# hpcaitech/Open-Sora

Hardware: NVIDIA H100
Metric: denoise-steps/sec STDiT3-XL/2 64x32x32 bf16 (higher is better)
Workload: dtype bf16

## Files before the change

### open-sora_b200/csrc/gemm_sm90.cu

```cuda
#include <stdlib.h>

#include <type_traits>

#include "common.cuh"
#include "tiles.cuh"
#include "wgmma.cuh"

namespace osb {

constexpr int kBlockM = 128;
constexpr int kBlockK = 64;
constexpr int kNumThreads = 384;
constexpr int kStageBudget = 200 * 1024;
constexpr int kSmemLimit = 227 * 1024;

enum { kPlain = 0, kConv = 1, kHeadTiles = 2, kLora = 3, kText = 4, kFp8 = 5, kFp8Blk = 6 };

struct Fp8BlockParams {
  int64_t a_ld, a_kstride;
  uint8_t* d8;
  float* d_scale;
  int64_t ldd8, ld_dscale;
};

// ... 13 lines not shown
struct HeadTileParams {
  uint8_t* base;
  int64_t kind_stride, head_stride;
  TileMap map;
  int32_t tile_bytes;
  int32_t heads, nkinds;
  uint32_t norm_mask, rope_mask;
  const __nv_bfloat16* norm_w[4];
  float eps;
  const float* cos;
  const float* sin;
};

struct ConvGeom {
  int32_t wt_log2, ht_log2;
  int32_t tiles_w, tiles_h, tiles_t, nb;
  int32_t w_out, h_out, t_out;
  int32_t sw, sh, st;
  int32_t kw_n, kh_n;
  int32_t cin_chunks;
};

__host__ __device__ constexpr bool staged_epilogue(int mode) { return mode == kPlain || mode == kConv || mode == kLora || mode == kFp8 || mode == kFp8Blk; }

template <int BLOCK_N, bool kStaged = false>
struct GemmCfg {
  static constexpr int A_BYTES = kBlockM * kBlockK * 2;
  static constexpr int B_BYTES = BLOCK_N * kBlockK * 2;
  static constexpr int STAGE_BYTES = A_BYTES + B_BYTES;
  static constexpr int EPI_BYTES = kStaged ? kBlockM * BLOCK_N * 2 : 0;
  static constexpr int RING_BUDGET = kStaged ? kSmemLimit - 1024 - 256 - EPI_BYTES : kStageBudget;
  static constexpr int STAGES_RAW = RING_BUDGET / STAGE_BYTES;
  static constexpr int STAGES = STAGES_RAW > 6 ? 6 : STAGES_RAW;
  static constexpr int NUM_BARS = 2 * STAGES + (kStaged ? 1 : 0);
  static constexpr int SMEM_BYTES = STAGES * STAGE_BYTES + EPI_BYTES + 1024 + 8 * NUM_BARS;
  static_assert(STAGES >= 2, "pipeline needs at least two stages");
  static_assert(SMEM_BYTES <= kSmemLimit, "shared memory");
  static_assert(B_BYTES % 1024 == 0, "W tile must keep 1024-byte swizzle-atom alignment");
  static_assert(BLOCK_N % 16 == 0 && BLOCK_N <= 256, "wgmma N");
  static_assert(!kStaged || BLOCK_N % 64 == 0, "the staged epilogue moves 64-column boxes");
};

template <int BLOCK_N, int kMode>
__global__ void __launch_bounds__(kNumThreads, 1)
gemm_bf16_kernel(const __grid_constant__ CUtensorMap tmap_a, const __grid_constant__ CUtensorMap tmap_w,
                 const GemmEpilogueParams p, const ConvGeom cg, const HeadTileParams ht,
                 const __grid_constant__ CUtensorMap tmap_u, const __grid_constant__ CUtensorMap tmap_lb,
                 const int32_t lora_k_blocks,
                 const float* a_scale, const float* w_scale,
                 const Fp8BlockParams fb,
                 const __grid_constant__ CUtensorMap tmap_r,
                 const __grid_constant__ CUtensorMap tmap_d) {
  constexpr bool kStaged = staged_epilogue(kMode);
  using Cfg = GemmCfg<BLOCK_N, kStaged>;
  constexpr int kStages = Cfg::STAGES;
  constexpr int kBK = (kMode == kFp8 || kMode == kFp8Blk) ? 2 * kBlockK : kBlockK;
  constexpr uint32_t kEpiBoxBytes = kBlockM * 128;

  extern __shared__ uint8_t smem_raw[];
  const uint32_t smem_base = (smem_u32(smem_raw) + 1023u) & ~1023u;
  const uint32_t epi_base = smem_base + kStages * Cfg::STAGE_BYTES;
  const uint32_t bar_base = epi_base + Cfg::EPI_BYTES;
  auto full_bar = [&](int s) { return bar_base + 8u * s; };
  auto empty_bar = [&](int s) { return bar_base + 8u * (kStages + s); };
  const uint32_t res_bar = bar_base + 8u * (2 * kStages);
  auto smem_a = [&](int s) { return smem_base + s * Cfg::STAGE_BYTES; };
  auto smem_b = [&](int s) { return smem_base + s * Cfg::STAGE_BYTES + Cfg::A_BYTES; };

  const int wg = threadIdx.x >> 7;
  const int tid_wg = threadIdx.x & 127;
  const int64_t num_n_blocks = (p.N + BLOCK_N - 1) / BLOCK_N;
  const int64_t m_blk = blockIdx.x / num_n_blocks, n_blk = blockIdx.x % num_n_blocks;
  const int64_t num_k_blocks = (p.K + kBK - 1) / kBK;
  const int64_t total_k_blocks = kMode == kLora ? num_k_blocks + lora_k_blocks : num_k_blocks;
  int n_i = 0, t0 = 0, h0 = 0, w0 = 0;
  if constexpr (kMode == kConv) {
    const int tw = (int)(m_blk % cg.tiles_w);
    const int th = (int)((m_blk / cg.tiles_w) % cg.tiles_h);
    const int tt = (int)((m_blk / ((int64_t)cg.tiles_w * cg.tiles_h)) % cg.tiles_t);
    n_i = (int)(m_blk / ((int64_t)cg.tiles_w * cg.tiles_h * cg.tiles_t));
    w0 = tw << cg.wt_log2;
    h0 = th << cg.ht_log2;
    t0 = tt * (128 >> (cg.wt_log2 + cg.ht_log2));
  }

  if (threadIdx.x == 0) {
    tma_prefetch_desc(&tmap_a);
    tma_prefetch_desc(&tmap_w);
    if constexpr (kMode == kLora) {
      tma_prefetch_desc(&tmap_u);
      tma_prefetch_desc(&tmap_lb);
    }
    if constexpr (kStaged) {
      if (p.R != nullptr) tma_prefetch_desc(&tmap_r);
      tma_prefetch_desc(&tmap_d);
      mbar_init(res_bar, 1);
    }
    for (int s = 0; s < kStages; ++s) {
      mbar_init(full_bar(s), 1);
      mbar_init(empty_bar(s), 2);
    }
    fence_barrier_init();
  }
  __syncthreads();
  pdl_wait();

  if (wg == 0) {
    if (tid_wg == 0) {
      const int32_t a_row = (int32_t)(m_blk * kBlockM);
      const int32_t w_row = (int32_t)(n_blk * BLOCK_N);
      if constexpr (kStaged) {
        if (p.R != nullptr) {
          const int live = (int)min((int64_t)(BLOCK_N / 64), (p.N - w_row + 63) / 64);
          mbar_expect_tx(res_bar, (uint32_t)live * kEpiBoxBytes);
          for (int c = 0; c < live; ++c) {
            if constexpr (kMode == kConv)
              tma_load_5d(&tmap_r, res_bar, epi_base + c * kEpiBoxBytes, w_row + 64 * c, w0, h0, t0, n_i);
            else
              tma_load_2d(&tmap_r, res_bar, epi_base + c * kEpiBoxBytes, w_row + 64 * c, a_row);
          }
        }
      }
      int stage = 0;
      uint32_t phase = 0;
      for (int64_t kb = 0; kb < num_k_blocks; ++kb) {
        mbar_wait_notrace(empty_bar(stage), phase ^ 1);
        const int32_t k0 = (int32_t)(kb * kBK);
        mbar_expect_tx(full_bar(stage), Cfg::STAGE_BYTES);
        if constexpr (kMode == kConv) {
          const int tap = (int)(kb / cg.cin_chunks);
          const int32_t ac = (int32_t)(kb - (int64_t)tap * cg.cin_chunks) * kBlockK;
          const int32_t aw = w0 * cg.sw + tap % cg.kw_n;
          const int32_t ah = h0 * cg.sh + (tap / cg.kw_n) % cg.kh_n;
          const int32_t at = t0 * cg.st + tap / (cg.kw_n * cg.kh_n);
          tma_load_5d(&tmap_a, full_bar(stage), smem_a(stage), ac, aw, ah, at, n_i);
        } else {
          tma_load_2d(&tmap_a, full_bar(stage), smem_a(stage), k0, a_row);
        }
        tma_load_2d(&tmap_w, full_bar(stage), smem_b(stage), k0, w_row);
        if (++stage == kStages) { stage = 0; phase ^= 1; }
      }
      if constexpr (kMode == kLora) {
        for (int32_t lk = 0; lk < lora_k_blocks; ++lk) {
          mbar_wait_notrace(empty_bar(stage), phase ^ 1);
          mbar_expect_tx(full_bar(stage), Cfg::STAGE_BYTES);
          tma_load_2d(&tmap_u, full_bar(stage), smem_a(stage), lk * kBlockK, a_row);
          tma_load_2d(&tmap_lb, full_bar(stage), smem_b(stage), lk * kBlockK, w_row);
          if (++stage == kStages) { stage = 0; phase ^= 1; }
        }
      }
      pdl_launch_dependents();
    }
    return;
  }

  const int cw = wg - 1;
  float acc[BLOCK_N / 2];
#pragma unroll
  for (int i = 0; i < BLOCK_N / 2; ++i) acc[i] = 0.f;
  if constexpr (kMode == kFp8 || kMode == kFp8Blk) {
    float part[BLOCK_N / 2];
#pragma unroll
    for (int i = 0; i < BLOCK_N / 2; ++i) part[i] = 0.f;
    const float* sa_row0 = a_scale;
    const float* sa_row1 = a_scale;
    if constexpr (kMode == kFp8Blk) {
      const int64_t r0 = m_blk * kBlockM + cw * 64 + (tid_wg >> 5) * 16 + ((tid_wg & 31) >> 2);
      sa_row0 = a_scale + min(r0, p.M - 1) * fb.a_ld;
      sa_row1 = a_scale + min(r0 + 8, p.M - 1) * fb.a_ld;
    }
    int stage = 0;
    uint32_t phase = 0;
    for (int64_t kb = 0; kb < total_k_blocks; ++kb) {
      float s0 = 1.f, s1 = 1.f;
      if constexpr (kMode == kFp8Blk) {
        s0 = __ldg(sa_row0 + kb * fb.a_kstride);
        s1 = __ldg(sa_row1 + kb * fb.a_kstride);
      }
      mbar_wait_notrace(full_bar(stage), phase);
      const uint64_t da = make_sw128_kmajor_desc(smem_a(stage) + (uint32_t)(cw * 64 * 128));
      const uint64_t db = make_sw128_kmajor_desc(smem_b(stage));
      wgmma_fence_regs(part);
      wgmma_fence();
#pragma unroll
      for (int k = 0; k < 4; ++k)
        WgmmaFp8<BLOCK_N>::mma(part, da + (uint64_t)(2 * k), db + (uint64_t)(2 * k), k > 0 ? 1u : 0u);
      wgmma_commit();
      wgmma_wait<0>();
      wgmma_fence_regs(part);
      if (tid_wg == 0) mbar_arrive(empty_bar(stage));
      if constexpr (kMode == kFp8Blk) {
#pragma unroll
        for (int j = 0; j < BLOCK_N / 8; ++j) {
          acc[4 * j] = fmaf(part[4 * j], s0, acc[4 * j]);
          acc[4 * j + 1] = fmaf(part[4 * j + 1], s0, acc[4 * j + 1]);
          acc[4 * j + 2] = fmaf(part[4 * j + 2], s1, acc[4 * j + 2]);
          acc[4 * j + 3] = fmaf(part[4 * j + 3], s1, acc[4 * j + 3]);
        }
      } else {
#pragma unroll
        for (int i = 0; i < BLOCK_N / 2; ++i) acc[i] += part[i];
      }
      if (++stage == kStages) { stage = 0; phase ^= 1; }
    }
  } else {
    int stage = 0, prev = 0;
    uint32_t phase = 0;
    for (int64_t kb = 0; kb < total_k_blocks; ++kb) {
      mbar_wait_notrace(full_bar(stage), phase);
      const uint64_t da = make_sw128_kmajor_desc(smem_a(stage) + (uint32_t)(cw * 64 * 128));
      const uint64_t db = make_sw128_kmajor_desc(smem_b(stage));
      wgmma_fence_regs(acc);
      wgmma_fence();
#pragma unroll
      for (int k = 0; k < kBlockK / 16; ++k)
        Wgmma<BLOCK_N>::mma(acc, da + (uint64_t)(2 * k), db + (uint64_t)(2 * k), (kb > 0 || k > 0) ? 1u : 0u);
      wgmma_commit();
      wgmma_wait<1>();
      wgmma_fence_regs(acc);
      if (kb > 0 && tid_wg == 0) mbar_arrive(empty_bar(prev));
      prev = stage;
      if (++stage == kStages) { stage = 0; phase ^= 1; }
    }
    wgmma_wait<0>();
    wgmma_fence_regs(acc);
  }

  const int warp_in = tid_wg >> 5, lane = tid_wg & 31;
  const int r_frag = cw * 64 + warp_in * 16 + (lane >> 2);
  const int c_frag = 2 * (lane & 3);

  if constexpr (kMode == kLora) {
    if (w_scale != nullptr) {
#pragma unroll
      for (int j = 0; j < BLOCK_N / 8; ++j) {
        const int64_t n = min(n_blk * BLOCK_N + 8 * j + c_frag, p.N - 2);
        const float2 cs = __ldg(reinterpret_cast<const float2*>(w_scale + n));
        acc[4 * j] *= cs.x;
        acc[4 * j + 1] *= cs.y;
        acc[4 * j + 2] *= cs.x;
        acc[4 * j + 3] *= cs.y;
      }
    }
  }

  if constexpr (kMode == kFp8Blk && BLOCK_N == 128) {
    if (p.epilogue == OSB_EPI_BIAS_GELU_TANH_FP8) {
      const int64_t n0 = n_blk * BLOCK_N + c_frag;
#pragma unroll
      for (int h = 0; h < 2; ++h) {
        const int64_t row = m_blk * kBlockM + r_frag + 8 * h;
        float amax = 0.f;
#pragma unroll
        for (int j = 0; j < BLOCK_N / 8; ++j) {
          const int64_t n = n0 + 8 * j;
          const float2 sw = __ldg(reinterpret_cast<const float2*>(w_scale + n));
          float v0 = acc[4 * j + 2 * h] * sw.x, v1 = acc[4 * j + 2 * h + 1] * sw.y;
          if (p.bias) {
            const float2 b = unpack_bf16x2(__ldg(reinterpret_cast<const uint32_t*>(p.bias + n)));
            v0 += b.x;
            v1 += b.y;
          }
          v0 = gelu_tanh(v0);
          v1 = gelu_tanh(v1);
          acc[4 * j + 2 * h] = v0;
          acc[4 * j + 2 * h + 1] = v1;
          amax = fmaxf(amax, fmaxf(fabsf(v0), fabsf(v1)));
        }
        amax = fmaxf(amax, __shfl_xor_sync(0xffffffffu, amax, 1));
        amax = fmaxf(amax, __shfl_xor_sync(0xffffffffu, amax, 2));
        const float s = amax > 0.f ? amax / 448.0f : 1.0f;
        if (row < p.M) {
          uint8_t* drow = fb.d8 + row * fb.ldd8;
#pragma unroll
          for (int j = 0; j < BLOCK_N / 8; ++j)
            *reinterpret_cast<uint16_t*>(drow + n0 + 8 * j) =
                (uint16_t)e4m3x2(acc[4 * j + 2 * h] / s, acc[4 * j + 2 * h + 1] / s);
          if (c_frag == 0) fb.d_scale[row * fb.ld_dscale + n_blk] = s;
        }
      }
      return;
    }
  }

  if constexpr (kMode == kHeadTiles) {
    constexpr int D = BLOCK_N / 2;
    using HT = HeadTileCfg<D>;
    constexpr int JH = D / 8;
    const int C = ht.heads * D;
    const uint32_t chunk_bytes = (uint32_t)ht.map.TR * 128u;
#pragma unroll
    for (int h = 0; h < 2; ++h) {
      const int64_t row = m_blk * kBlockM + r_frag + 8 * h;
      const bool row_ok = row < p.M;
      uint32_t pos = 0, tile_i = 0, seq;
      int r = 0;
      if (row_ok) {
        const uint32_t row32 = (uint32_t)row;
        if (ht.map.mode == 0) {
          seq = row32 / (uint32_t)ht.map.L;
          pos = row32 - seq * (uint32_t)ht.map.L;
        } else {
          const uint32_t ts = (uint32_t)ht.map.T * (uint32_t)ht.map.S;
          const uint32_t b = row32 / ts;
          const uint32_t rem = row32 - b * ts;
          pos = rem / (uint32_t)ht.map.S;
          seq = b * (uint32_t)ht.map.S + (rem - pos * (uint32_t)ht.map.S);
        }
        if (ht.map.G > 1) {
          tile_i = seq / (uint32_t)ht.map.G;
          r = (int)((seq - tile_i * (uint32_t)ht.map.G) * (uint32_t)ht.map.L + pos);
        } else {
          const uint32_t jt = pos / (uint32_t)ht.map.TR;
          tile_i = seq * (uint32_t)ht.map.tps + jt;
          r = (int)(pos - jt * (uint32_t)ht.map.TR);
        }
      }
#pragma unroll
      for (int hh = 0; hh < 2; ++hh) {
        const int64_t col0 = n_blk * BLOCK_N + hh * D;
        if (col0 >= p.N) continue;
        const int kidx = (int)((uint32_t)col0 / (uint32_t)C);
        const int head = (int)((uint32_t)col0 - (uint32_t)kidx * (uint32_t)C) / D;
        const int kind = kidx % ht.nkinds;
        float x[JH][2];
#pragma unroll
        for (int j = 0; j < JH; ++j) {
          x[j][0] = acc[4 * (hh * JH + j) + 2 * h];
          x[j][1] = acc[4 * (hh * JH + j) + 2 * h + 1];
          if (p.bias) {
            const float2 b = unpack_bf16x2(__ldg(reinterpret_cast<const uint32_t*>(p.bias + col0 + 8 * j + c_frag)));
            x[j][0] += b.x;
            x[j][1] += b.y;
          }
        }
        if ((ht.norm_mask >> kind) & 1u) {
          float ss = 0.f;
#pragma unroll
          for (int j = 0; j < JH; ++j) ss += x[j][0] * x[j][0] + x[j][1] * x[j][1];
          ss += __shfl_xor_sync(0xffffffffu, ss, 1);
          ss += __shfl_xor_sync(0xffffffffu, ss, 2);
          const float rs = rsqrtf(ss * (1.0f / D) + ht.eps);
          const __nv_bfloat16* w = kind == 0 ? ht.norm_w[0] : (kind == 1 ? ht.norm_w[1] : (kind == 2 ? ht.norm_w[2] : ht.norm_w[3]));
#pragma unroll
          for (int j = 0; j < JH; ++j) {
            const float2 f = unpack_bf16x2(__ldg(reinterpret_cast<const uint32_t*>(w + 8 * j + c_frag)));
            x[j][0] *= rs * f.x;
            x[j][1] *= rs * f.y;
          }
        }
        if (!row_ok) continue;
        if ((ht.rope_mask >> kind) & 1u) {
#pragma unroll
          for (int j = 0; j < JH; ++j) {
            const int64_t i = (int64_t)pos * (D / 2) + (8 * j + c_frag) / 2;
            const float cc = __ldg(ht.cos + i), sn = __ldg(ht.sin + i);
            const float a = x[j][0], b = x[j][1];
            x[j][0] = a * cc - b * sn;
            x[j][1] = b * cc + a * sn;
          }
        }
        uint8_t* dst = ht.base + (int64_t)kidx * ht.kind_stride + (int64_t)head * ht.head_stride + (int64_t)tile_i * ht.tile_bytes;
#pragma unroll
        for (int j = 0; j < JH; ++j)
          *reinterpret_cast<uint32_t*>(dst + tile_unit_off<HT::MAIN>(r, j, chunk_bytes) + c_frag * 2) = pack_bf16x2(x[j][0], x[j][1]);
        if constexpr (HT::UP > HT::U)
          *reinterpret_cast<uint32_t*>(dst + tile_unit_off<HT::MAIN>(r, HT::U, chunk_bytes) + c_frag * 2) = 0u;
      }
    }
  } else if constexpr (kMode == kText) {
#pragma unroll
    for (int h = 0; h < 2; ++h) {
      const int64_t row = m_blk * kBlockM + r_frag + 8 * h;
      if (row >= p.M) continue;
      __nv_bfloat16* drow = p.D + row * p.ldd;
#pragma unroll
      for (int j = 0; j < BLOCK_N / 8; ++j) {
        const int64_t n = n_blk * BLOCK_N + 8 * j + c_frag;
        if (n >= p.N) continue;
        float v0 = acc[4 * j + 2 * h], v1 = acc[4 * j + 2 * h + 1];
        if (p.bias) {
          const float2 b = unpack_bf16x2(__ldg(reinterpret_cast<const uint32_t*>(p.bias + n)));
          v0 += b.x;
          v1 += b.y;
        }
        if (p.epilogue == OSB_EPI_GATED_GELU) {
          drow[n >> 1] = __float2bfloat16_rn(gelu_tanh(v0) * v1);
        } else {
          v0 = v0 / (1.0f + __expf(-1.702f * v0));
          v1 = v1 / (1.0f + __expf(-1.702f * v1));
          *reinterpret_cast<uint32_t*>(drow + n) = pack_bf16x2(v0, v1);
        }
      }
    }
  } else {
    static_assert(kStaged, "every other mode has its own epilogue");
    const float* gate_row[2] = {nullptr, nullptr};
    float sa[2] = {0.f, 0.f};
    if constexpr (kMode != kConv) {
      const uint32_t group_rows32 = (uint32_t)(p.group_rows > 0xffffffffll ? 0xffffffffu : p.group_rows);
#pragma unroll
      for (int h = 0; h < 2; ++h) {
        const int64_t row = min(m_blk * kBlockM + r_frag + 8 * h, p.M - 1);
        if (p.epilogue == OSB_EPI_BIAS_GATE_RES && p.gate != nullptr) {
          int64_t gi = (uint32_t)row / group_rows32;
          if (p.mod_index) gi = p.mod_index[gi];
          gate_row[h] = p.gate + gi * p.gate_stride;
        }
        if constexpr (kMode == kFp8) sa[h] = __ldg(a_scale + row);
      }
    }
    uint8_t* const epi = smem_raw + (epi_base - smem_u32(smem_raw));
    const bool gate_res = p.epilogue == OSB_EPI_BIAS_GATE_RES;
    if (!gate_res) gate_row[0] = gate_row[1] = nullptr;
    const bool has_res = gate_res && p.R != nullptr;
    if (p.R != nullptr) mbar_wait_notrace(res_bar, 0);
    auto body = [&](auto gelu) {
#pragma unroll
      for (int j = 0; j < BLOCK_N / 8; ++j) {
        const int64_t n = min(n_blk * BLOCK_N + 8 * j + c_frag, p.N - 2);
        float2 sw = make_float2(1.f, 1.f), b = make_float2(-0.f, -0.f);
        if constexpr (kMode == kFp8 || kMode == kFp8Blk) sw = __ldg(reinterpret_cast<const float2*>(w_scale + n));
        if (p.bias) b = unpack_bf16x2(__ldg(reinterpret_cast<const uint32_t*>(p.bias + n)));
#pragma unroll
        for (int h = 0; h < 2; ++h) {
          const int li = r_frag + 8 * h;
          uint32_t* const cell = reinterpret_cast<uint32_t*>(epi + (j >> 3) * kEpiBoxBytes + li * 128 +
                                                             (((j & 7) ^ (li & 7)) << 4) + c_frag * 2);
          float v0 = acc[4 * j + 2 * h], v1 = acc[4 * j + 2 * h + 1];
          if constexpr (kMode == kFp8) {
            v0 = __fmul_rn(v0, __fmul_rn(sa[h], sw.x));
            v1 = __fmul_rn(v1, __fmul_rn(sa[h], sw.y));
          } else if constexpr (kMode == kFp8Blk) {
            v0 = __fmul_rn(v0, sw.x);
            v1 = __fmul_rn(v1, sw.y);
          }
          v0 = __fadd_rn(v0, b.x);
          v1 = __fadd_rn(v1, b.y);
          if constexpr (decltype(gelu)::value) {
            v0 = gelu_tanh(v0);
            v1 = gelu_tanh(v1);
          } else {
            const float2 g = gate_row[h] ? __ldg(reinterpret_cast<const float2*>(gate_row[h] + n)) : make_float2(1.f, 1.f);
            const float2 rv = has_res ? unpack_bf16x2(*cell) : make_float2(-0.f, -0.f);
            v0 = __fadd_rn(__fmul_rn(v0, g.x), rv.x);
            v1 = __fadd_rn(__fmul_rn(v1, g.y), rv.y);
          }
          *cell = pack_bf16x2(v0, v1);
        }
      }
    };
    if (p.epilogue == OSB_EPI_BIAS_GELU_TANH)
      body(std::true_type{});
    else
      body(std::false_type{});
    fence_proxy_async_smem();
    named_barrier_sync(1, 256);
    if (threadIdx.x == 128) {
      const int32_t n0 = (int32_t)(n_blk * BLOCK_N);
      const int live = (int)min((int64_t)(BLOCK_N / 64), (p.N - n0 + 63) / 64);
      for (int c = 0; c < live; ++c) {
        if constexpr (kMode == kConv)
          tma_store_5d(&tmap_d, epi_base + c * kEpiBoxBytes, n0 + 64 * c, w0, h0, t0, n_i);
        else
          tma_store_2d(&tmap_d, epi_base + c * kEpiBoxBytes, n0 + 64 * c, (int32_t)(m_blk * kBlockM));
      }
      bulk_commit_group();
      bulk_wait_group_read_all();
    }
  }
}

template <int BLOCK_N, int kMode>
static int launch_kernel(const CUtensorMap& ta, const CUtensorMap& tw, const GemmEpilogueParams& p, const ConvGeom& cg,
                         const HeadTileParams& ht, int64_t tiles, cudaStream_t stream, const CUtensorMap* tu = nullptr,
                         const CUtensorMap* tlb = nullptr, int32_t lora_k_blocks = 0, const float* a_scale = nullptr,
                         const float* w_scale = nullptr, const Fp8BlockParams& fb = Fp8BlockParams{},
                         const CUtensorMap* tr = nullptr, const CUtensorMap* td = nullptr) {
  if (tiles >= (1ll << 31)) { set_error("osb gemm: too many output tiles (%lld)", (long long)tiles); return OSB_ERR_UNSUPPORTED; }
  cudaLaunchAttribute attr[2];
  cudaLaunchConfig_t cfg = launch_config(dim3((unsigned)tiles), dim3(kNumThreads),
                                         GemmCfg<BLOCK_N, staged_epilogue(kMode)>::SMEM_BYTES, stream, attr);
  OSB_CHECK_CUDA(cudaLaunchKernelEx(&cfg, gemm_bf16_kernel<BLOCK_N, kMode>, ta, tw, p, cg, ht, tu ? *tu : ta,
                                    tlb ? *tlb : tw, lora_k_blocks, a_scale, w_scale, fb, tr ? *tr : ta, td ? *td : ta));
  count_launch();
  return OSB_OK;
}

static int make_epilogue_maps(const GemmEpilogueParams& p, CUtensorMap* tr, CUtensorMap* td) {
  if (int rc = make_tmap_2d_bf16(td, p.D, p.M, p.N, p.ldd, kBlockM, 64)) return rc;
  if (p.R != nullptr) return make_tmap_2d_bf16(tr, p.R, p.M, p.N, p.ldr, kBlockM, 64);
  *tr = *td;
  return OSB_OK;
}

template <int D>
static int launch_gemm_ht(const osb_gemm_args& a, const HeadTileParams& ht, cudaStream_t stream) {
  constexpr int BLOCK_N = 2 * D;
  CUtensorMap ta, tw;
  int rc = make_tmap_2d_bf16(&ta, a.A, a.M, a.K, a.lda, kBlockM, kBlockK);
  if (rc) return rc;
  rc = make_tmap_2d_bf16(&tw, a.W, a.N, a.K, a.ldw, BLOCK_N, kBlockK);
  if (rc) return rc;
  GemmEpilogueParams p = {};
  p.bias = static_cast<const __nv_bfloat16*>(a.bias);
  p.M = a.M; p.N = a.N; p.K = a.K;
  p.group_rows = a.M;
  p.epilogue = OSB_EPI_BIAS;
  const int64_t tiles = ((a.M + kBlockM - 1) / kBlockM) * ((a.N + BLOCK_N - 1) / BLOCK_N);
  ConvGeom cg = {};
  return launch_kernel<BLOCK_N, kHeadTiles>(ta, tw, p, cg, ht, tiles, stream);
}

template <int BLOCK_N>
// ... 408 lines not shown
```

Measured before the change: 11.22.

## Make SM90 GEMM persistent with overlapped epilogue TMA stores and register reallocation

Turns the one-tile-per-CTA GEMM into a persistent kernel whose grid is capped at the SM count, except for head-tile mode. The producer warp streams k-blocks across successive tiles, a second producer lane issues the output TMA stores, and two new mbarriers hand the staging buffer back and forth so the next tile's mainloop can overlap the previous tile's store and residual load. Producer registers are reduced and consumer registers raised with setmaxnreg. This is meant to cut launch and tail overhead and hide epilogue latency, at the cost of more complex synchronisation and a risk of serialising on the single epilogue buffer.

```diff
diff --git a/open-sora_b200/csrc/gemm_sm90.cu b/open-sora_b200/csrc/gemm_sm90.cu
--- a/open-sora_b200/csrc/gemm_sm90.cu
+++ b/open-sora_b200/csrc/gemm_sm90.cu
@@ -69,7 +69,7 @@
   static constexpr int RING_BUDGET = kStaged ? kSmemLimit - 1024 - 256 - EPI_BYTES : kStageBudget;
   static constexpr int STAGES_RAW = RING_BUDGET / STAGE_BYTES;
   static constexpr int STAGES = STAGES_RAW > 6 ? 6 : STAGES_RAW;
-  static constexpr int NUM_BARS = 2 * STAGES + (kStaged ? 1 : 0);
+  static constexpr int NUM_BARS = 2 * STAGES + (kStaged ? 3 : 0);
   static constexpr int SMEM_BYTES = STAGES * STAGE_BYTES + EPI_BYTES + 1024 + 8 * NUM_BARS;
   static_assert(STAGES >= 2, "pipeline needs at least two stages");
   static_assert(SMEM_BYTES <= kSmemLimit, "shared memory");
@@ -101,25 +101,43 @@
   auto full_bar = [&](int s) { return bar_base + 8u * s; };
   auto empty_bar = [&](int s) { return bar_base + 8u * (kStages + s); };
   const uint32_t res_bar = bar_base + 8u * (2 * kStages);
+  const uint32_t epi_full = res_bar + 8u;
+  const uint32_t epi_free = res_bar + 16u;
   auto smem_a = [&](int s) { return smem_base + s * Cfg::STAGE_BYTES; };
   auto smem_b = [&](int s) { return smem_base + s * Cfg::STAGE_BYTES + Cfg::A_BYTES; };
 
   const int wg = threadIdx.x >> 7;
   const int tid_wg = threadIdx.x & 127;
   const int64_t num_n_blocks = (p.N + BLOCK_N - 1) / BLOCK_N;
-  const int64_t m_blk = blockIdx.x / num_n_blocks, n_blk = blockIdx.x % num_n_blocks;
+  const int64_t num_m_blocks = kMode == kConv ? (int64_t)cg.nb * cg.tiles_t * cg.tiles_h * cg.tiles_w : (p.M + kBlockM - 1) / kBlockM;
+  const int64_t num_tiles = num_m_blocks * num_n_blocks;
   const int64_t num_k_blocks = (p.K + kBK - 1) / kBK;
   const int64_t total_k_blocks = kMode == kLora ? num_k_blocks + lora_k_blocks : num_k_blocks;
-  int n_i = 0, t0 = 0, h0 = 0, w0 = 0;
-  if constexpr (kMode == kConv) {
-    const int tw = (int)(m_blk % cg.tiles_w);
-    const int th = (int)((m_blk / cg.tiles_w) % cg.tiles_h);
-    const int tt = (int)((m_blk / ((int64_t)cg.tiles_w * cg.tiles_h)) % cg.tiles_t);
-    n_i = (int)(m_blk / ((int64_t)cg.tiles_w * cg.tiles_h * cg.tiles_t));
-    w0 = tw << cg.wt_log2;
-    h0 = th << cg.ht_log2;
-    t0 = tt * (128 >> (cg.wt_log2 + cg.ht_log2));
-  }
+  bool epi_buffer = kStaged;
+  if constexpr (kMode == kFp8Blk && BLOCK_N == 128) epi_buffer = p.epilogue != OSB_EPI_BIAS_GELU_TANH_FP8;
+
+  struct Tile {
+    int64_t m_blk, n_blk;
+    int n_i, t0, h0, w0;
+  };
+  auto tile_at = [&](int64_t tile) {
+    Tile c;
+    const uint32_t mb = (uint32_t)tile / (uint32_t)num_n_blocks;
+    c.m_blk = mb;
+    c.n_blk = (uint32_t)tile - mb * (uint32_t)num_n_blocks;
+    c.n_i = c.t0 = c.h0 = c.w0 = 0;
+    if constexpr (kMode == kConv) {
+      const uint32_t mh = mb / (uint32_t)cg.tiles_w, mt = mh / (uint32_t)cg.tiles_h;
+      const int tw = (int)(mb - mh * (uint32_t)cg.tiles_w);
+      const int th = (int)(mh - mt * (uint32_t)cg.tiles_h);
+      c.n_i = (int)(mt / (uint32_t)cg.tiles_t);
+      const int tt = (int)(mt - (uint32_t)c.n_i * (uint32_t)cg.tiles_t);
+      c.w0 = tw << cg.wt_log2;
+      c.h0 = th << cg.ht_log2;
+      c.t0 = tt * (128 >> (cg.wt_log2 + cg.ht_log2));
+    }
+    return c;
+  };
 
   if (threadIdx.x == 0) {
     tma_prefetch_desc(&tmap_a);
@@ -132,6 +150,8 @@
       if (p.R != nullptr) tma_prefetch_desc(&tmap_r);
       tma_prefetch_desc(&tmap_d);
       mbar_init(res_bar, 1);
+      mbar_init(epi_full, 1);
+      mbar_init(epi_free, 1);
     }
     for (int s = 0; s < kStages; ++s) {
       mbar_init(full_bar(s), 1);
@@ -143,367 +163,395 @@
   pdl_wait();
 
   if (wg == 0) {
+    asm volatile("setmaxnreg.dec.sync.aligned.u32 40;\n" ::: "memory");
     if (tid_wg == 0) {
-      const int32_t a_row = (int32_t)(m_blk * kBlockM);
-      const int32_t w_row = (int32_t)(n_blk * BLOCK_N);
-      if constexpr (kStaged) {
-        if (p.R != nullptr) {
-          const int live = (int)min((int64_t)(BLOCK_N / 64), (p.N - w_row + 63) / 64);
-          mbar_expect_tx(res_bar, (uint32_t)live * kEpiBoxBytes);
-          for (int c = 0; c < live; ++c) {
-            if constexpr (kMode == kConv)
-              tma_load_5d(&tmap_r, res_bar, epi_base + c * kEpiBoxBytes, w_row + 64 * c, w0, h0, t0, n_i);
-            else
-              tma_load_2d(&tmap_r, res_bar, epi_base + c * kEpiBoxBytes, w_row + 64 * c, a_row);
-          }
-        }
-      }
       int stage = 0;
       uint32_t phase = 0;
-      for (int64_t kb = 0; kb < num_k_blocks; ++kb) {
-        mbar_wait_notrace(empty_bar(stage), phase ^ 1);
-        const int32_t k0 = (int32_t)(kb * kBK);
-        mbar_expect_tx(full_bar(stage), Cfg::STAGE_BYTES);
-        if constexpr (kMode == kConv) {
-          const int tap = (int)(kb / cg.cin_chunks);
-          const int32_t ac = (int32_t)(kb - (int64_t)tap * cg.cin_chunks) * kBlockK;
-          const int32_t aw = w0 * cg.sw + tap % cg.kw_n;
-          const int32_t ah = h0 * cg.sh + (tap / cg.kw_n) % cg.kh_n;
-          const int32_t at = t0 * cg.st + tap / (cg.kw_n * cg.kh_n);
-          tma_load_5d(&tmap_a, full_bar(stage), smem_a(stage), ac, aw, ah, at, n_i);
-        } else {
-          tma_load_2d(&tmap_a, full_bar(stage), smem_a(stage), k0, a_row);
-        }
-        tma_load_2d(&tmap_w, full_bar(stage), smem_b(stage), k0, w_row);
-        if (++stage == kStages) { stage = 0; phase ^= 1; }
-      }
-      if constexpr (kMode == kLora) {
-        for (int32_t lk = 0; lk < lora_k_blocks; ++lk) {
+      uint32_t t = 0;
+      for (int64_t tile = blockIdx.x; tile < num_tiles; tile += gridDim.x, ++t) {
+        const Tile c = tile_at(tile);
+        const int32_t a_row = (int32_t)(c.m_blk * kBlockM);
+        const int32_t w_row = (int32_t)(c.n_blk * BLOCK_N);
+        bool res_pending = kStaged && p.R != nullptr;
+        const uint32_t prev_free = (t & 1u) ^ 1u;
+        auto load_res = [&]() {
+          if constexpr (kStaged) {
+            const int live = (int)min((int64_t)(BLOCK_N / 64), (p.N - w_row + 63) / 64);
+            mbar_expect_tx(res_bar, (uint32_t)live * kEpiBoxBytes);
+            for (int i = 0; i < live; ++i) {
+              if constexpr (kMode == kConv)
+                tma_load_5d(&tmap_r, res_bar, epi_base + i * kEpiBoxBytes, w_row + 64 * i, c.w0, c.h0, c.t0, c.n_i);
+              else
+                tma_load_2d(&tmap_r, res_bar, epi_base + i * kEpiBoxBytes, w_row + 64 * i, a_row);
+            }
+          }
+          res_pending = false;
+        };
+        int chunk = 0, tap_w = 0, tap_h = 0, tap_t = 0;
+        for (int32_t kb = 0;; ++kb) {
+          const bool done = kb == (int32_t)total_k_blocks;
+          if (res_pending && (done || mbar_test_wait(epi_free, prev_free))) {
+            mbar_wait_notrace(epi_free, prev_free);
+            load_res();
+          }
+          if (done) break;
           mbar_wait_notrace(empty_bar(stage), phase ^ 1);
           mbar_expect_tx(full_bar(stage), Cfg::STAGE_BYTES);
-          tma_load_2d(&tmap_u, full_bar(stage), smem_a(stage), lk * kBlockK, a_row);
-          tma_load_2d(&tmap_lb, full_bar(stage), smem_b(stage), lk * kBlockK, w_row);
+          if (kMode == kLora && kb >= num_k_blocks) {
+            const int32_t lk = (kb - (int32_t)num_k_blocks) * kBlockK;
+            tma_load_2d(&tmap_u, full_bar(stage), smem_a(stage), lk, a_row);
+            tma_load_2d(&tmap_lb, full_bar(stage), smem_b(stage), lk, w_row);
+          } else {
+            const int32_t k0 = kb * kBK;
+            if constexpr (kMode == kConv) {
+              tma_load_5d(&tmap_a, full_bar(stage), smem_a(stage), chunk * kBlockK, c.w0 * cg.sw + tap_w,
+                          c.h0 * cg.sh + tap_h, c.t0 * cg.st + tap_t, c.n_i);
+              if (++chunk == cg.cin_chunks) {
+                chunk = 0;
+                if (++tap_w == cg.kw_n) {
+                  tap_w = 0;
+                  if (++tap_h == cg.kh_n) { tap_h = 0; ++tap_t; }
+                }
+              }
+            } else {
+              tma_load_2d(&tmap_a, full_bar(stage), smem_a(stage), k0, a_row);
+            }
+            tma_load_2d(&tmap_w, full_bar(stage), smem_b(stage), k0, w_row);
+          }
           if (++stage == kStages) { stage = 0; phase ^= 1; }
         }
       }
       pdl_launch_dependents();
+    } else if (tid_wg == 32 && epi_buffer) {
+      uint32_t t = 0;
+      for (int64_t tile = blockIdx.x; tile < num_tiles; tile += gridDim.x, ++t) {
+        const Tile c = tile_at(tile);
+        const int32_t n0 = (int32_t)(c.n_blk * BLOCK_N);
+        const int live = (int)min((int64_t)(BLOCK_N / 64), (p.N - n0 + 63) / 64);
+        mbar_wait_notrace(epi_full, t & 1u);
+        for (int i = 0; i < live; ++i) {
+          if constexpr (kMode == kConv)
+            tma_store_5d(&tmap_d, epi_base + i * kEpiBoxBytes, n0 + 64 * i, c.w0, c.h0, c.t0, c.n_i);
+          else
+            tma_store_2d(&tmap_d, epi_base + i * kEpiBoxBytes, n0 + 64 * i, (int32_t)(c.m_blk * kBlockM));
+        }
+        bulk_commit_group();
+        bulk_wait_group_read_all();
+        mbar_arrive(epi_free);
+      }
     }
     return;
   }
 
+  asm volatile("setmaxnreg.inc.sync.aligned.u32 232;\n" ::: "memory");
   const int cw = wg - 1;
-  float acc[BLOCK_N / 2];
-#pragma unroll
-  for (int i = 0; i < BLOCK_N / 2; ++i) acc[i] = 0.f;
-  if constexpr (kMode == kFp8 || kMode == kFp8Blk) {
-    float part[BLOCK_N / 2];
-#pragma unroll
-    for (int i = 0; i < BLOCK_N / 2; ++i) part[i] = 0.f;
-    const float* sa_row0 = a_scale;
-    const float* sa_row1 = a_scale;
-    if constexpr (kMode == kFp8Blk) {
-      const int64_t r0 = m_blk * kBlockM + cw * 64 + (tid_wg >> 5) * 16 + ((tid_wg & 31) >> 2);
-      sa_row0 = a_scale + min(r0, p.M - 1) * fb.a_ld;
-      sa_row1 = a_scale + min(r0 + 8, p.M - 1) * fb.a_ld;
-    }
-    int stage = 0;
-    uint32_t phase = 0;
-    for (int64_t kb = 0; kb < total_k_blocks; ++kb) {
-      float s0 = 1.f, s1 = 1.f;
-      if constexpr (kMode == kFp8Blk) {
-        s0 = __ldg(sa_row0 + kb * fb.a_kstride);
-        s1 = __ldg(sa_row1 + kb * fb.a_kstride);
-      }
-      mbar_wait_notrace(full_bar(stage), phase);
-      const uint64_t da = make_sw128_kmajor_desc(smem_a(stage) + (uint32_t)(cw * 64 * 128));
-      const uint64_t db = make_sw128_kmajor_desc(smem_b(stage));
-      wgmma_fence_regs(part);
-      wgmma_fence();
-#pragma unroll
-      for (int k = 0; k < 4; ++k)
-        WgmmaFp8<BLOCK_N>::mma(part, da + (uint64_t)(2 * k), db + (uint64_t)(2 * k), k > 0 ? 1u : 0u);
-      wgmma_commit();
-      wgmma_wait<0>();
-      wgmma_fence_regs(part);
-      if (tid_wg == 0) mbar_arrive(empty_bar(stage));
-      if constexpr (kMode == kFp8Blk) {
-#pragma unroll
-        for (int j = 0; j < BLOCK_N / 8; ++j) {
-          acc[4 * j] = fmaf(part[4 * j], s0, acc[4 * j]);
-          acc[4 * j + 1] = fmaf(part[4 * j + 1], s0, acc[4 * j + 1]);
-          acc[4 * j + 2] = fmaf(part[4 * j + 2], s1, acc[4 * j + 2]);
-          acc[4 * j + 3] = fmaf(part[4 * j + 3], s1, acc[4 * j + 3]);
-        }
-      } else {
-#pragma unroll
-        for (int i = 0; i < BLOCK_N / 2; ++i) acc[i] += part[i];
-      }
-      if (++stage == kStages) { stage = 0; phase ^= 1; }
-    }
-  } else {
-    int stage = 0, prev = 0;
-    uint32_t phase = 0;
-    for (int64_t kb = 0; kb < total_k_blocks; ++kb) {
-      mbar_wait_notrace(full_bar(stage), phase);
-      const uint64_t da = make_sw128_kmajor_desc(smem_a(stage) + (uint32_t)(cw * 64 * 128));
-      const uint64_t db = make_sw128_kmajor_desc(smem_b(stage));
-      wgmma_fence_regs(acc);
-      wgmma_fence();
-#pragma unroll
-      for (int k = 0; k < kBlockK / 16; ++k)
-        Wgmma<BLOCK_N>::mma(acc, da + (uint64_t)(2 * k), db + (uint64_t)(2 * k), (kb > 0 || k > 0) ? 1u : 0u);
-      wgmma_commit();
-      wgmma_wait<1>();
-      wgmma_fence_regs(acc);
-      if (kb > 0 && tid_wg == 0) mbar_arrive(empty_bar(prev));
-      prev = stage;
-      if (++stage == kStages) { stage = 0; phase ^= 1; }
-    }
-    wgmma_wait<0>();
-    wgmma_fence_regs(acc);
-  }
-
   const int warp_in = tid_wg >> 5, lane = tid_wg & 31;
   const int r_frag = cw * 64 + warp_in * 16 + (lane >> 2);
   const int c_frag = 2 * (lane & 3);
-
-  if constexpr (kMode == kLora) {
-    if (w_scale != nullptr) {
-#pragma unroll
-      for (int j = 0; j < BLOCK_N / 8; ++j) {
-        const int64_t n = min(n_blk * BLOCK_N + 8 * j + c_frag, p.N - 2);
-        const float2 cs = __ldg(reinterpret_cast<const float2*>(w_scale + n));
-        acc[4 * j] *= cs.x;
-        acc[4 * j + 1] *= cs.y;
-        acc[4 * j + 2] *= cs.x;
-        acc[4 * j + 3] *= cs.y;
+  int stage = 0, prev = 0;
+  uint32_t phase = 0;
+  uint32_t t = 0;
+  for (int64_t tile = blockIdx.x; tile < num_tiles; tile += gridDim.x, ++t) {
+    const Tile c = tile_at(tile);
+    const int64_t m_blk = c.m_blk, n_blk = c.n_blk;
+    float acc[BLOCK_N / 2];
+#pragma unroll
+    for (int i = 0; i < BLOCK_N / 2; ++i) acc[i] = 0.f;
+    if constexpr (kMode == kFp8 || kMode == kFp8Blk) {
+      float part[BLOCK_N / 2];
+#pragma unroll
+      for (int i = 0; i < BLOCK_N / 2; ++i) part[i] = 0.f;
+      const float* sa_row0 = a_scale;
+      const float* sa_row1 = a_scale;
+      if constexpr (kMode == kFp8Blk) {
+        const int64_t r0 = m_blk * kBlockM + r_frag;
+        sa_row0 = a_scale + min(r0, p.M - 1) * fb.a_ld;
+        sa_row1 = a_scale + min(r0 + 8, p.M - 1) * fb.a_ld;
+      }
+      for (int64_t kb = 0; kb < total_k_blocks; ++kb) {
+        float s0 = 1.f, s1 = 1.f;
+        if constexpr (kMode == kFp8Blk) {
+          s0 = __ldg(sa_row0 + kb * fb.a_kstride);
+          s1 = __ldg(sa_row1 + kb * fb.a_kstride);
+        }
+        mbar_wait_notrace(full_bar(stage), phase);
+        const uint64_t da = make_sw128_kmajor_desc(smem_a(stage) + (uint32_t)(cw * 64 * 128));
+        const uint64_t db = make_sw128_kmajor_desc(smem_b(stage));
+        wgmma_fence_regs(part);
+        wgmma_fence();
+#pragma unroll
+        for (int k = 0; k < 4; ++k)
+          WgmmaFp8<BLOCK_N>::mma(part, da + (uint64_t)(2 * k), db + (uint64_t)(2 * k), k > 0 ? 1u : 0u);
+        wgmma_commit();
+        wgmma_wait<0>();
+        wgmma_fence_regs(part);
+        if (tid_wg == 0) mbar_arrive(empty_bar(stage));
+        if constexpr (kMode == kFp8Blk) {
+#pragma unroll
+          for (int j = 0; j < BLOCK_N / 8; ++j) {
+            acc[4 * j] = fmaf(part[4 * j], s0, acc[4 * j]);
+            acc[4 * j + 1] = fmaf(part[4 * j + 1], s0, acc[4 * j + 1]);
+            acc[4 * j + 2] = fmaf(part[4 * j + 2], s1, acc[4 * j + 2]);
+            acc[4 * j + 3] = fmaf(part[4 * j + 3], s1, acc[4 * j + 3]);
+          }
+        } else {
+#pragma unroll
+          for (int i = 0; i < BLOCK_N / 2; ++i) acc[i] += part[i];
+        }
+        if (++stage == kStages) { stage = 0; phase ^= 1; }
+      }
+    } else {
+      for (int64_t kb = 0; kb < total_k_blocks; ++kb) {
+        mbar_wait_notrace(full_bar(stage), phase);
+        const uint64_t da = make_sw128_kmajor_desc(smem_a(stage) + (uint32_t)(cw * 64 * 128));
+        const uint64_t db = make_sw128_kmajor_desc(smem_b(stage));
+        wgmma_fence_regs(acc);
+        wgmma_fence();
+#pragma unroll
+        for (int k = 0; k < kBlockK / 16; ++k)
+          Wgmma<BLOCK_N>::mma(acc, da + (uint64_t)(2 * k), db + (uint64_t)(2 * k), (kb > 0 || k > 0) ? 1u : 0u);
+        wgmma_commit();
+        wgmma_wait<1>();
+        wgmma_fence_regs(acc);
+        if (kb > 0 && tid_wg == 0) mbar_arrive(empty_bar(prev));
+        prev = stage;
+        if (++stage == kStages) { stage = 0; phase ^= 1; }
+      }
+      wgmma_wait<0>();
+      wgmma_fence_regs(acc);
+      if (tid_wg == 0) mbar_arrive(empty_bar(prev));
+    }
+
+    if constexpr (kMode == kLora) {
+      if (w_scale != nullptr) {
+#pragma unroll
+        for (int j = 0; j < BLOCK_N / 8; ++j) {
+          const int64_t n = min(n_blk * BLOCK_N + 8 * j + c_frag, p.N - 2);
+          const float2 cs = __ldg(reinterpret_cast<const float2*>(w_scale + n));
+          acc[4 * j] *= cs.x;
+          acc[4 * j + 1] *= cs.y;
+          acc[4 * j + 2] *= cs.x;
+          acc[4 * j + 3] *= cs.y;
+        }
       }
     }
-  }
-
-  if constexpr (kMode == kFp8Blk && BLOCK_N == 128) {
-    if (p.epilogue == OSB_EPI_BIAS_GELU_TANH_FP8) {
-      const int64_t n0 = n_blk * BLOCK_N + c_frag;
+
+    if constexpr (kMode == kFp8Blk && BLOCK_N == 128) {
+      if (p.epilogue == OSB_EPI_BIAS_GELU_TANH_FP8) {
+        const int64_t n0 = n_blk * BLOCK_N + c_frag;
+#pragma unroll
+        for (int h = 0; h < 2; ++h) {
+          const int64_t row = m_blk * kBlockM + r_frag + 8 * h;
+          float amax = 0.f;
+#pragma unroll
+          for (int j = 0; j < BLOCK_N / 8; ++j) {
+            const int64_t n = n0 + 8 * j;
+            const float2 sw = __ldg(reinterpret_cast<const float2*>(w_scale + n));
+            float v0 = acc[4 * j + 2 * h] * sw.x, v1 = acc[4 * j + 2 * h + 1] * sw.y;
+            if (p.bias) {
+              const float2 b = unpack_bf16x2(__ldg(reinterpret_cast<const uint32_t*>(p.bias + n)));
+              v0 += b.x;
+              v1 += b.y;
+            }
+            v0 = gelu_tanh(v0);
+            v1 = gelu_tanh(v1);
+            acc[4 * j + 2 * h] = v0;
+            acc[4 * j + 2 * h + 1] = v1;
+            amax = fmaxf(amax, fmaxf(fabsf(v0), fabsf(v1)));
+          }
+          amax = fmaxf(amax, __shfl_xor_sync(0xffffffffu, amax, 1));
+          amax = fmaxf(amax, __shfl_xor_sync(0xffffffffu, amax, 2));
+          const float s = amax > 0.f ? amax / 448.0f : 1.0f;
+          if (row < p.M) {
+            uint8_t* drow = fb.d8 + row * fb.ldd8;
+#pragma unroll
+            for (int j = 0; j < BLOCK_N / 8; ++j)
+              *reinterpret_cast<uint16_t*>(drow + n0 + 8 * j) =
+                  (uint16_t)e4m3x2(acc[4 * j + 2 * h] / s, acc[4 * j + 2 * h + 1] / s);
+            if (c_frag == 0) fb.d_scale[row * fb.ld_dscale + n_blk] = s;
+          }
+        }
+        continue;
+      }
+    }
+
+    if constexpr (kMode == kHeadTiles) {
+      constexpr int D = BLOCK_N / 2;
+      using HT = HeadTileCfg<D>;
+      constexpr int JH = D / 8;
+      const int C = ht.heads * D;
+      const uint32_t chunk_bytes = (uint32_t)ht.map.TR * 128u;
 #pragma unroll
       for (int h = 0; h < 2; ++h) {
         const int64_t row = m_blk * kBlockM + r_frag + 8 * h;
-        float amax = 0.f;
+        const bool row_ok = row < p.M;
+        uint32_t pos = 0, tile_i = 0, seq;
+        int r = 0;
+        if (row_ok) {
+          const uint32_t row32 = (uint32_t)row;
+          if (ht.map.mode == 0) {
+            seq = row32 / (uint32_t)ht.map.L;
+            pos = row32 - seq * (uint32_t)ht.map.L;
+          } else {
+            const uint32_t ts = (uint32_t)ht.map.T * (uint32_t)ht.map.S;
+            const uint32_t b = row32 / ts;
+            const uint32_t rem = row32 - b * ts;
+            pos = rem / (uint32_t)ht.map.S;
+            seq = b * (uint32_t)ht.map.S + (rem - pos * (uint32_t)ht.map.S);
+          }
+          if (ht.map.G > 1) {
+            tile_i = seq / (uint32_t)ht.map.G;
+            r = (int)((seq - tile_i * (uint32_t)ht.map.G) * (uint32_t)ht.map.L + pos);
+          } else {
+            const uint32_t jt = pos / (uint32_t)ht.map.TR;
+            tile_i = seq * (uint32_t)ht.map.tps + jt;
+            r = (int)(pos - jt * (uint32_t)ht.map.TR);
+          }
+        }
+#pragma unroll
+        for (int hh = 0; hh < 2; ++hh) {
+          const int64_t col0 = n_blk * BLOCK_N + hh * D;
+          if (col0 >= p.N) continue;
+          const int kidx = (int)((uint32_t)col0 / (uint32_t)C);
+          const int head = (int)((uint32_t)col0 - (uint32_t)kidx * (uint32_t)C) / D;
+          const int kind = kidx % ht.nkinds;
+          float x[JH][2];
+#pragma unroll
+          for (int j = 0; j < JH; ++j) {
+            x[j][0] = acc[4 * (hh * JH + j) + 2 * h];
+            x[j][1] = acc[4 * (hh * JH + j) + 2 * h + 1];
+            if (p.bias) {
+              const float2 b = unpack_bf16x2(__ldg(reinterpret_cast<const uint32_t*>(p.bias + col0 + 8 * j + c_frag)));
+              x[j][0] += b.x;
+              x[j][1] += b.y;
+            }
+          }
+          if ((ht.norm_mask >> kind) & 1u) {
+            float ss = 0.f;
+#pragma unroll
+            for (int j = 0; j < JH; ++j) ss += x[j][0] * x[j][0] + x[j][1] * x[j][1];
+            ss += __shfl_xor_sync(0xffffffffu, ss, 1);
+            ss += __shfl_xor_sync(0xffffffffu, ss, 2);
+            const float rs = rsqrtf(ss * (1.0f / D) + ht.eps);
+            const __nv_bfloat16* w = kind == 0 ? ht.norm_w[0] : (kind == 1 ? ht.norm_w[1] : (kind == 2 ? ht.norm_w[2] : ht.norm_w[3]));
+#pragma unroll
+            for (int j = 0; j < JH; ++j) {
+              const float2 f = unpack_bf16x2(__ldg(reinterpret_cast<const uint32_t*>(w + 8 * j + c_frag)));
+              x[j][0] *= rs * f.x;
+              x[j][1] *= rs * f.y;
+            }
+          }
+          if (!row_ok) continue;
+          if ((ht.rope_mask >> kind) & 1u) {
+#pragma unroll
+            for (int j = 0; j < JH; ++j) {
+              const int64_t i = (int64_t)pos * (D / 2) + (8 * j + c_frag) / 2;
+              const float cc = __ldg(ht.cos + i), sn = __ldg(ht.sin + i);
+              const float a = x[j][0], b = x[j][1];
+              x[j][0] = a * cc - b * sn;
+              x[j][1] = b * cc + a * sn;
+            }
+          }
+          uint8_t* dst = ht.base + (int64_t)kidx * ht.kind_stride + (int64_t)head * ht.head_stride + (int64_t)tile_i * ht.tile_bytes;
+#pragma unroll
+          for (int j = 0; j < JH; ++j)
+            *reinterpret_cast<uint32_t*>(dst + tile_unit_off<HT::MAIN>(r, j, chunk_bytes) + c_frag * 2) = pack_bf16x2(x[j][0], x[j][1]);
+          if constexpr (HT::UP > HT::U)
+            *reinterpret_cast<uint32_t*>(dst + tile_unit_off<HT::MAIN>(r, HT::U, chunk_bytes) + c_frag * 2) = 0u;
+        }
+      }
+    } else if constexpr (kMode == kText) {
+#pragma unroll
+      for (int h = 0; h < 2; ++h) {
+        const int64_t row = m_blk * kBlockM + r_frag + 8 * h;
+        if (row >= p.M) continue;
+        __nv_bfloat16* drow = p.D + row * p.ldd;
 #pragma unroll
         for (int j = 0; j < BLOCK_N / 8; ++j) {
-          const int64_t n = n0 + 8 * j;
-          const float2 sw = __ldg(reinterpret_cast<const float2*>(w_scale + n));
-          float v0 = acc[4 * j + 2 * h] * sw.x, v1 = acc[4 * j + 2 * h + 1] * sw.y;
+          const int64_t n = n_blk * BLOCK_N + 8 * j + c_frag;
+          if (n >= p.N) continue;
+          float v0 = acc[4 * j + 2 * h], v1 = acc[4 * j + 2 * h + 1];
           if (p.bias) {
             const float2 b = unpack_bf16x2(__ldg(reinterpret_cast<const uint32_t*>(p.bias + n)));
             v0 += b.x;
             v1 += b.y;
           }
-          v0 = gelu_tanh(v0);
-          v1 = gelu_tanh(v1);
-          acc[4 * j + 2 * h] = v0;
-          acc[4 * j + 2 * h + 1] = v1;
-          amax = fmaxf(amax, fmaxf(fabsf(v0), fabsf(v1)));
-        }
-        amax = fmaxf(amax, __shfl_xor_sync(0xffffffffu, amax, 1));
-        amax = fmaxf(amax, __shfl_xor_sync(0xffffffffu, amax, 2));
-        const float s = amax > 0.f ? amax / 448.0f : 1.0f;
-        if (row < p.M) {
-          uint8_t* drow = fb.d8 + row * fb.ldd8;
-#pragma unroll
-          for (int j = 0; j < BLOCK_N / 8; ++j)
-            *reinterpret_cast<uint16_t*>(drow + n0 + 8 * j) =
-                (uint16_t)e4m3x2(acc[4 * j + 2 * h] / s, acc[4 * j + 2 * h + 1] / s);
-          if (c_frag == 0) fb.d_scale[row * fb.ld_dscale + n_blk] = s;
+          if (p.epilogue == OSB_EPI_GATED_GELU) {
+            drow[n >> 1] = __float2bfloat16_rn(gelu_tanh(v0) * v1);
+          } else {
+            v0 = v0 / (1.0f + __expf(-1.702f * v0));
+            v1 = v1 / (1.0f + __expf(-1.702f * v1));
+            *reinterpret_cast<uint32_t*>(drow + n) = pack_bf16x2(v0, v1);
+          }
         }
       }
-      return;
-    }
-  }
-
-  if constexpr (kMode == kHeadTiles) {
-    constexpr int D = BLOCK_N / 2;
-    using HT = HeadTileCfg<D>;
-    constexpr int JH = D / 8;
-    const int C = ht.heads * D;
-    const uint32_t chunk_bytes = (uint32_t)ht.map.TR * 128u;
-#pragma unroll
-    for (int h = 0; h < 2; ++h) {
-      const int64_t row = m_blk * kBlockM + r_frag + 8 * h;
-      const bool row_ok = row < p.M;
-      uint32_t pos = 0, tile_i = 0, seq;
-      int r = 0;
-      if (row_ok) {
-        const uint32_t row32 = (uint32_t)row;
-        if (ht.map.mode == 0) {
-          seq = row32 / (uint32_t)ht.map.L;
-          pos = row32 - seq * (uint32_t)ht.map.L;
-        } else {
-          const uint32_t ts = (uint32_t)ht.map.T * (uint32_t)ht.map.S;
-          const uint32_t b = row32 / ts;
-          const uint32_t rem = row32 - b * ts;
-          pos = rem / (uint32_t)ht.map.S;
-          seq = b * (uint32_t)ht.map.S + (rem - pos * (uint32_t)ht.map.S);
-        }
-        if (ht.map.G > 1) {
-          tile_i = seq / (uint32_t)ht.map.G;
-          r = (int)((seq - tile_i * (uint32_t)ht.map.G) * (uint32_t)ht.map.L + pos);
-        } else {
-          const uint32_t jt = pos / (uint32_t)ht.map.TR;
-          tile_i = seq * (uint32_t)ht.map.tps + jt;
-          r = (int)(pos - jt * (uint32_t)ht.map.TR);
+    } else {
+      static_assert(kStaged, "every other mode has its own epilogue");
+      const float* gate_row[2] = {nullptr, nullptr};
+      float sa[2] = {0.f, 0.f};
+      if constexpr (kMode != kConv) {
+        const uint32_t group_rows32 = (uint32_t)(p.group_rows > 0xffffffffll ? 0xffffffffu : p.group_rows);
+#pragma unroll
+        for (int h = 0; h < 2; ++h) {
+          const int64_t row = min(m_blk * kBlockM + r_frag + 8 * h, p.M - 1);
+          if (p.epilogue == OSB_EPI_BIAS_GATE_RES && p.gate != nullptr) {
+            int64_t gi = (uint32_t)row / group_rows32;
+            if (p.mod_index) gi = p.mod_index[gi];
+            gate_row[h] = p.gate + gi * p.gate_stride;
+          }
+          if constexpr (kMode == kFp8) sa[h] = __ldg(a_scale + row);
         }
       }
-#pragma unroll
-      for (int hh = 0; hh < 2; ++hh) {
-        const int64_t col0 = n_blk * BLOCK_N + hh * D;
-        if (col0 >= p.N) continue;
-        const int kidx = (int)((uint32_t)col0 / (uint32_t)C);
-        const int head = (int)((uint32_t)col0 - (uint32_t)kidx * (uint32_t)C) / D;
-        const int kind = kidx % ht.nkinds;
-        float x[JH][2];
-#pragma unroll
-        for (int j = 0; j < JH; ++j) {
-          x[j][0] = acc[4 * (hh * JH + j) + 2 * h];
-          x[j][1] = acc[4 * (hh * JH + j) + 2 * h + 1];
-          if (p.bias) {
-            const float2 b = unpack_bf16x2(__ldg(reinterpret_cast<const uint32_t*>(p.bias + col0 + 8 * j + c_frag)));
-            x[j][0] += b.x;
-            x[j][1] += b.y;
+      uint8_t* const epi = smem_raw + (epi_base - smem_u32(smem_raw));
+      const bool gate_res = p.epilogue == OSB_EPI_BIAS_GATE_RES;
+      if (!gate_res) gate_row[0] = gate_row[1] = nullptr;
+      const bool has_res = gate_res && p.R != nullptr;
+      if (p.R != nullptr)
+        mbar_wait_notrace(res_bar, t & 1u);
+      else
+        mbar_wait_notrace(epi_free, (t & 1u) ^ 1u);
+      auto body = [&](auto gelu) {
+#pragma unroll
+        for (int j = 0; j < BLOCK_N / 8; ++j) {
+          const int64_t n = min(n_blk * BLOCK_N + 8 * j + c_frag, p.N - 2);
+          float2 sw = make_float2(1.f, 1.f), b = make_float2(-0.f, -0.f);
+          if constexpr (kMode == kFp8 || kMode == kFp8Blk) sw = __ldg(reinterpret_cast<const float2*>(w_scale + n));
+          if (p.bias) b = unpack_bf16x2(__ldg(reinterpret_cast<const uint32_t*>(p.bias + n)));
+#pragma unroll
+          for (int h = 0; h < 2; ++h) {
+            const int li = r_frag + 8 * h;
+            uint32_t* const cell = reinterpret_cast<uint32_t*>(epi + (j >> 3) * kEpiBoxBytes + li * 128 +
+                                                               (((j & 7) ^ (li & 7)) << 4) + c_frag * 2);
+            float v0 = acc[4 * j + 2 * h], v1 = acc[4 * j + 2 * h + 1];
+            if constexpr (kMode == kFp8) {
+              v0 = __fmul_rn(v0, __fmul_rn(sa[h], sw.x));
+              v1 = __fmul_rn(v1, __fmul_rn(sa[h], sw.y));
+            } else if constexpr (kMode == kFp8Blk) {
+              v0 = __fmul_rn(v0, sw.x);
+              v1 = __fmul_rn(v1, sw.y);
+            }
+            v0 = __fadd_rn(v0, b.x);
+            v1 = __fadd_rn(v1, b.y);
+            if constexpr (decltype(gelu)::value) {
+              v0 = gelu_tanh(v0);
+              v1 = gelu_tanh(v1);
+            } else {
+              const float2 g = gate_row[h] ? __ldg(reinterpret_cast<const float2*>(gate_row[h] + n)) : make_float2(1.f, 1.f);
+              const float2 rv = has_res ? unpack_bf16x2(*cell) : make_float2(-0.f, -0.f);
+              v0 = __fadd_rn(__fmul_rn(v0, g.x), rv.x);
+              v1 = __fadd_rn(__fmul_rn(v1, g.y), rv.y);
+            }
+            *cell = pack_bf16x2(v0, v1);
           }
         }
-        if ((ht.norm_mask >> kind) & 1u) {
-          float ss = 0.f;
-#pragma unroll
-          for (int j = 0; j < JH; ++j) ss += x[j][0] * x[j][0] + x[j][1] * x[j][1];
-          ss += __shfl_xor_sync(0xffffffffu, ss, 1);
-          ss += __shfl_xor_sync(0xffffffffu, ss, 2);
-          const float rs = rsqrtf(ss * (1.0f / D) + ht.eps);
-          const __nv_bfloat16* w = kind == 0 ? ht.norm_w[0] : (kind == 1 ? ht.norm_w[1] : (kind == 2 ? ht.norm_w[2] : ht.norm_w[3]));
-#pragma unroll
-          for (int j = 0; j < JH; ++j) {
-            const float2 f = unpack_bf16x2(__ldg(reinterpret_cast<const uint32_t*>(w + 8 * j + c_frag)));
-            x[j][0] *= rs * f.x;
-            x[j][1] *= rs * f.y;
-          }
-        }
-        if (!row_ok) continue;
-        if ((ht.rope_mask >> kind) & 1u) {
-#pragma unroll
-          for (int j = 0; j < JH; ++j) {
-            const int64_t i = (int64_t)pos * (D / 2) + (8 * j + c_frag) / 2;
-            const float cc = __ldg(ht.cos + i), sn = __ldg(ht.sin + i);
-            const float a = x[j][0], b = x[j][1];
-            x[j][0] = a * cc - b * sn;
-            x[j][1] = b * cc + a * sn;
-          }
-        }
-        uint8_t* dst = ht.base + (int64_t)kidx * ht.kind_stride + (int64_t)head * ht.head_stride + (int64_t)tile_i * ht.tile_bytes;
-#pragma unroll
-        for (int j = 0; j < JH; ++j)
-          *reinterpret_cast<uint32_t*>(dst + tile_unit_off<HT::MAIN>(r, j, chunk_bytes) + c_frag * 2) = pack_bf16x2(x[j][0], x[j][1]);
-        if constexpr (HT::UP > HT::U)
-          *reinterpret_cast<uint32_t*>(dst + tile_unit_off<HT::MAIN>(r, HT::U, chunk_bytes) + c_frag * 2) = 0u;
-      }
-    }
-  } else if constexpr (kMode == kText) {
-#pragma unroll
-    for (int h = 0; h < 2; ++h) {
-      const int64_t row = m_blk * kBlockM + r_frag + 8 * h;
-      if (row >= p.M) continue;
-      __nv_bfloat16* drow = p.D + row * p.ldd;
-#pragma unroll
-      for (int j = 0; j < BLOCK_N / 8; ++j) {
-        const int64_t n = n_blk * BLOCK_N + 8 * j + c_frag;
-        if (n >= p.N) continue;
-        float v0 = acc[4 * j + 2 * h], v1 = acc[4 * j + 2 * h + 1];
-        if (p.bias) {
-          const float2 b = unpack_bf16x2(__ldg(reinterpret_cast<const uint32_t*>(p.bias + n)));
-          v0 += b.x;
-          v1 += b.y;
-        }
-        if (p.epilogue == OSB_EPI_GATED_GELU) {
-          drow[n >> 1] = __float2bfloat16_rn(gelu_tanh(v0) * v1);
-        } else {
-          v0 = v0 / (1.0f + __expf(-1.702f * v0));
-          v1 = v1 / (1.0f + __expf(-1.702f * v1));
-          *reinterpret_cast<uint32_t*>(drow + n) = pack_bf16x2(v0, v1);
-        }
-      }
-    }
-  } else {
-    static_assert(kStaged, "every other mode has its own epilogue");
-    const float* gate_row[2] = {nullptr, nullptr};
-    float sa[2] = {0.f, 0.f};
-    if constexpr (kMode != kConv) {
-      const uint32_t group_rows32 = (uint32_t)(p.group_rows > 0xffffffffll ? 0xffffffffu : p.group_rows);
-#pragma unroll
-      for (int h = 0; h < 2; ++h) {
-        const int64_t row = min(m_blk * kBlockM + r_frag + 8 * h, p.M - 1);
-        if (p.epilogue == OSB_EPI_BIAS_GATE_RES && p.gate != nullptr) {
-          int64_t gi = (uint32_t)row / group_rows32;
-          if (p.mod_index) gi = p.mod_index[gi];
-          gate_row[h] = p.gate + gi * p.gate_stride;
-        }
-        if constexpr (kMode == kFp8) sa[h] = __ldg(a_scale + row);
-      }
-    }
-    uint8_t* const epi = smem_raw + (epi_base - smem_u32(smem_raw));
-    const bool gate_res = p.epilogue == OSB_EPI_BIAS_GATE_RES;
-    if (!gate_res) gate_row[0] = gate_row[1] = nullptr;
-    const bool has_res = gate_res && p.R != nullptr;
-    if (p.R != nullptr) mbar_wait_notrace(res_bar, 0);
-    auto body = [&](auto gelu) {
-#pragma unroll
-      for (int j = 0; j < BLOCK_N / 8; ++j) {
-        const int64_t n = min(n_blk * BLOCK_N + 8 * j + c_frag, p.N - 2);
-        float2 sw = make_float2(1.f, 1.f), b = make_float2(-0.f, -0.f);
-        if constexpr (kMode == kFp8 || kMode == kFp8Blk) sw = __ldg(reinterpret_cast<const float2*>(w_scale + n));
-        if (p.bias) b = unpack_bf16x2(__ldg(reinterpret_cast<const uint32_t*>(p.bias + n)));
-#pragma unroll
-        for (int h = 0; h < 2; ++h) {
-          const int li = r_frag + 8 * h;
-          uint32_t* const cell = reinterpret_cast<uint32_t*>(epi + (j >> 3) * kEpiBoxBytes + li * 128 +
-                                                             (((j & 7) ^ (li & 7)) << 4) + c_frag * 2);
-          float v0 = acc[4 * j + 2 * h], v1 = acc[4 * j + 2 * h + 1];
-          if constexpr (kMode == kFp8) {
-            v0 = __fmul_rn(v0, __fmul_rn(sa[h], sw.x));
-            v1 = __fmul_rn(v1, __fmul_rn(sa[h], sw.y));
-          } else if constexpr (kMode == kFp8Blk) {
-            v0 = __fmul_rn(v0, sw.x);
-            v1 = __fmul_rn(v1, sw.y);
-          }
-          v0 = __fadd_rn(v0, b.x);
-          v1 = __fadd_rn(v1, b.y);
-          if constexpr (decltype(gelu)::value) {
-            v0 = gelu_tanh(v0);
-            v1 = gelu_tanh(v1);
-          } else {
-            const float2 g = gate_row[h] ? __ldg(reinterpret_cast<const float2*>(gate_row[h] + n)) : make_float2(1.f, 1.f);
-            const float2 rv = has_res ? unpack_bf16x2(*cell) : make_float2(-0.f, -0.f);
-            v0 = __fadd_rn(__fmul_rn(v0, g.x), rv.x);
-            v1 = __fadd_rn(__fmul_rn(v1, g.y), rv.y);
-          }
-          *cell = pack_bf16x2(v0, v1);
-        }
-      }
-    };
-    if (p.epilogue == OSB_EPI_BIAS_GELU_TANH)
-      body(std::true_type{});
-    else
-      body(std::false_type{});
-    fence_proxy_async_smem();
-    named_barrier_sync(1, 256);
-    if (threadIdx.x == 128) {
-      const int32_t n0 = (int32_t)(n_blk * BLOCK_N);
-      const int live = (int)min((int64_t)(BLOCK_N / 64), (p.N - n0 + 63) / 64);
-      for (int c = 0; c < live; ++c) {
-        if constexpr (kMode == kConv)
-          tma_store_5d(&tmap_d, epi_base + c * kEpiBoxBytes, n0 + 64 * c, w0, h0, t0, n_i);
-        else
-          tma_store_2d(&tmap_d, epi_base + c * kEpiBoxBytes, n0 + 64 * c, (int32_t)(m_blk * kBlockM));
-      }
-      bulk_commit_group();
-      bulk_wait_group_read_all();
+      };
+      if (p.epilogue == OSB_EPI_BIAS_GELU_TANH)
+        body(std::true_type{});
+      else
+        body(std::false_type{});
+      fence_proxy_async_smem();
+      named_barrier_sync(1, 256);
+      if (threadIdx.x == 128) mbar_arrive(epi_full);
     }
   }
 }
@@ -516,7 +564,8 @@
                          const CUtensorMap* tr = nullptr, const CUtensorMap* td = nullptr) {
   if (tiles >= (1ll << 31)) { set_error("osb gemm: too many output tiles (%lld)", (long long)tiles); return OSB_ERR_UNSUPPORTED; }
   cudaLaunchAttribute attr[2];
-  cudaLaunchConfig_t cfg = launch_config(dim3((unsigned)tiles), dim3(kNumThreads),
+  const int64_t grid = (kMode == kHeadTiles || tiles < sm_count()) ? tiles : sm_count();
+  cudaLaunchConfig_t cfg = launch_config(dim3((unsigned)grid), dim3(kNumThreads),
                                          GemmCfg<BLOCK_N, staged_epilogue(kMode)>::SMEM_BYTES, stream, attr);
   OSB_CHECK_CUDA(cudaLaunchKernelEx(&cfg, gemm_bf16_kernel<BLOCK_N, kMode>, ta, tw, p, cg, ht, tu ? *tu : ta,
                                     tlb ? *tlb : tw, lora_k_blocks, a_scale, w_scale, fb, tr ? *tr : ta, td ? *td : ta));
```

Measured after the change: 11.53, median of 6. +2.7%, better.
